# phylovi/libsbn

Measured on AMD Instinct MI355X. Metric: tree log-likelihoods+gradients/sec (batched), higher is better.
Workload: dtype f64; 1 GPU; DS1 27 taxa x 934 site patterns x 1000 trees per step over 1 GPU(s), JC69+weibull+4 (K=4), phylo_gradients: logL + branch + site gradients; trees_total=1000, trees_per_gpu=1000, taxa=27, patterns=934, categories=4, parallelism=single GPU

## Files before the change

libsbn_amd/csrc/kernels_finalize.hip:

```cpp
#include <hip/hip_runtime.h>

#include <algorithm>
#include <cstdlib>
#include <string>

#include "mi_phylo_device_utils.h"
#include "mi_phylo_kernels.h"

namespace miphylo {

namespace {
using namespace dev;

__device__ __forceinline__ void reduce_tiles_body(const ReduceArgs& a, const int b, double* red_lds ,
                                                  double* keep = nullptr) {
  __shared__ double llw[4];
  const int lane = threadIdx.x & 63, wv = threadIdx.x >> 6;
  const int N2 = 2 * a.N;
  const int W = a.g_width ? a.g_width : N2;
  const int t = b < a.T ? b : b - a.T;
  const bool positional = b < a.Eg && a.g_width;
  const int mcount = positional ? a.macro_count[t] : 0;
  double llp = 0;
  for (int i = threadIdx.x; i < a.ll_used.of(b); i += 256) llp += a.ll_part[(size_t)b * a.ll_tiles + i];
// ... 507 lines not shown
    if (a.rooted) finalize_body_t<true, true>(a, t, fin_lds, keep);
    else finalize_body_t<true, false>(a, t, fin_lds, keep);
  } else {
    if (a.rooted) finalize_body_t<false, true>(a, t, fin_lds, keep);
    else finalize_body_t<false, false>(a, t, fin_lds, keep);
  }
}

__global__ __launch_bounds__(64) void finalize_kernel(FinalizeArgs a) {
  extern __shared__ double fin_lds[];
  finalize_body(a, blockIdx.x, fin_lds);
}

__global__ __launch_bounds__(256) void reduce_finalize_kernel(ReduceArgs ra, FinalizeArgs fa) {
  extern __shared__ double rf_lds[];
  if (threadIdx.x == 0 && fa.clear_ready) fa.clear_ready[(size_t)blockIdx.x * kReadyStride] = 0;
  double* keep = rf_lds + ra.keep_offset;
  reduce_tiles_body(ra, blockIdx.x, rf_lds, keep);
  __threadfence_block();
  __syncthreads();
  if (threadIdx.x >= 64) return;
  finalize_body(fa, blockIdx.x, rf_lds, keep);
}

__device__ __forceinline__ double hess_wave_share(const double* src, int W, int g_tiles, int col, int wv) {
  double s0 = 0, s1 = 0;
  int i = wv;
  for (; i + 4 < g_tiles; i += 8) {
    s0 += src[(size_t)i * W + col];
    s1 += src[(size_t)(i + 4) * W + col];
  }
  if (i < g_tiles) s0 += src[(size_t)i * W + col];
  return s0 + s1;
}
__global__ __launch_bounds__(256) void hessian_finalize_kernel(HessFinalizeArgs a) {
  __shared__ double llw[4];
  const int t = blockIdx.x, lane = threadIdx.x & 63, wv = threadIdx.x >> 6;
// ... 92 lines not shown
  hipLaunchKernelGGL(reduce_tiles_kernel, dim3(a.E), dim3(256), sizeof(double) * 4 * W, s, a);
}
static size_t finalize_lds_bytes(const FinalizeArgs& a) {
  return sizeof(double) * (a.rooted ? 22 * (size_t)a.n : 6 * (size_t)a.n);
}
void launch_reduce_finalize(const ReduceArgs& ra_in, const FinalizeArgs& fa_in, hipStream_t s) {
  FinalizeArgs fa = fa_in;
  ReduceArgs ra = ra_in;
  const size_t W = ra.g_width ? ra.g_width : 2 * (size_t)ra.N;
  const size_t fin = finalize_lds_bytes(fa);
  fa.use_lds = fin <= 48 * 1024;
  const size_t work = std::max(sizeof(double) * 4 * W, fa.use_lds ? fin : 0);
  ra.keep_offset = (int)(work / sizeof(double));
  const size_t lds = work + sizeof(double) * (2 * (size_t)ra.N + 1);
  allow_large_lds(reinterpret_cast<const void*>(reduce_finalize_kernel), lds);
  hipLaunchKernelGGL(reduce_finalize_kernel, dim3(fa.T), dim3(256), lds, s, ra, fa);
}
void launch_finalize(const FinalizeArgs& a_in, hipStream_t s) {
  FinalizeArgs a = a_in;
  const size_t lds = sizeof(double) * (a.rooted ? 22 * (size_t)a.n : 6 * (size_t)a.n);
  a.use_lds = lds <= 48 * 1024;
  hipLaunchKernelGGL(finalize_kernel, dim3(a.T), dim3(64), a.use_lds ? lds : 0, s, a);
}

}
```

libsbn_amd/csrc/kernels_setup.hip:

```cpp
#include <hip/hip_runtime.h>

#include <algorithm>
#include <cstdlib>
#include <string>

#include "mi_phylo_device_utils.h"
#include "mi_phylo_kernels.h"
#include "mi_phylo_setup_device.h"
#include "mi_phylo_macro_slots_device.h"

namespace miphylo {

namespace {
using namespace dev;


__global__ __launch_bounds__(64) void tree_setup_kernel(TreeSetupArgs a, ModelSetupArgs ms) {
  if ((int)blockIdx.x >= a.T) {
    model_setup_thread(ms, ((int)blockIdx.x - a.T) * 64 + (int)threadIdx.x);
    return;
  }
  extern __shared__ int32_t ts_lds[];
  const int t = blockIdx.x;
  const int lane = threadIdx.x;
  const int n = a.n, N = 2 * n - 1;
  const int nodes_in = a.rooted ? N : N - 1;
  const int32_t* par_in = a.parent_ids + (size_t)t * (nodes_in - 1);
  int32_t* maxleaf = a.use_lds ? ts_lds : a.scratch + (size_t)t * 13 * N;
  int32_t* cnt = maxleaf + N;
  int32_t* kids = cnt + N;
  int32_t* c0 = kids + 3 * N;
  int32_t* c1 = c0 + N;
  int32_t* label = c1 + N;
  int32_t* slot = label + N;
  int32_t* stack = slot + N;
  int32_t* par = stack + 2 * N;
  __shared__ int ok_flag;
  SchedEntry* sched = a.sched + (size_t)t * (n - 1);
// ... 147 lines not shown
__device__ __forceinline__ uint64_t up_word(int cls, int label, int isz, int mxl) {
  return (1ull << 63) | ((uint64_t)cls << 56) | ((uint64_t)label << 48) | ((uint64_t)isz << 20) | (uint64_t)mxl;
}
__device__ __forceinline__ int up_cls(uint64_t w) { return (int)(w >> 56) & 3; }
__device__ __forceinline__ int up_label(uint64_t w) { return (int)(w >> 48) & 0xff; }
__device__ __forceinline__ int up_isz(uint64_t w) { return (int)(w >> 20) & 0xfffff; }
__device__ __forceinline__ int up_mxl(uint64_t w) { return (int)w & 0xfffff; }
__global__ __launch_bounds__(kSetupMaxThreads) void tree_setup_wg_kernel(TreeSetupArgs a, ModelSetupArgs ms) {
  const int tid = threadIdx.x, nthreads = blockDim.x;
  if ((int)blockIdx.x >= a.T) {
    model_setup_thread(ms, ((int)blockIdx.x - a.T) * nthreads + tid);
    return;
  }
  extern __shared__ int32_t ts_lds[];
  __shared__ int flag_bad, flag_arity, used_max, chunk_tot[64], ok_flag;
  const int t = blockIdx.x;
  const int n = a.n, N = 2 * n - 1;
  const int nodes_in = a.rooted ? N : N - 1, root_in = nodes_in - 1;
  const int32_t* par_in = a.parent_ids + (size_t)t * (nodes_in - 1);
#define TS_LDS(T) volatile __attribute__((address_space(3))) T*
  typedef __attribute__((address_space(3))) int32_t* ts_lds_base;
  const ts_lds_base ts3 = (ts_lds_base)ts_lds;
  TS_LDS(int4) kid = (TS_LDS(int4))ts3;
  TS_LDS(uint64_t) W = (TS_LDS(uint64_t))(ts3 + 4 * N);
  TS_LDS(uint64_t) D = W + N;
  TS_LDS(int2) cc = (TS_LDS(int2))(D + N);
  TS_LDS(int2) up = cc + N;
  TS_LDS(int32_t) par = (TS_LDS(int32_t))(up + N);
  TS_LDS(int32_t) sslot = par + N;
#undef TS_LDS
  int32_t* kid_i = ts_lds;
// ... 248 lines not shown
  if (a.arena_macros) {
    __syncthreads();
    macro_slots_wg_body(ts_lds, a.macros, a.arena_macros, macro_M, n, t, a.slot_need, a.arena_sure, a.status);
  }
}


template <int NB>
__global__ __launch_bounds__(64) void tree_setup_small_kernel(TreeSetupArgs a, ModelSetupArgs ms) {
  if ((int)blockIdx.x >= a.T) {
    model_setup_thread(ms, ((int)blockIdx.x - a.T) * 64 + (int)threadIdx.x);
    return;
  }
  __shared__ int tree_lds[kSmallTreeLdsInts * NB];
  SmallTree<NB> tree;
  small_tree_build<NB>(a, blockIdx.x, threadIdx.x, tree, tree_lds);
  small_tree_store<NB>(a, blockIdx.x, threadIdx.x, tree);
}

constexpr int kTransitionBlock = 256;
__global__ __launch_bounds__(kTransitionBlock) void transition_kernel(TransitionArgs a) {
  __shared__ double stage[kTransitionBlock * 17];
  const long per = (long)a.K * (a.N - 1);
  const long first = (long)blockIdx.x * kTransitionBlock + (long)a.eval_base * per;
  const long idx = first + threadIdx.x;
  const long total = (long)(a.eval_base + a.E) * per;
  {
    const long last = (first + kTransitionBlock - 1 < total ? first + kTransitionBlock - 1 : total - 1);
    if (first / per >= a.ev_skip_begin && last / per < a.ev_skip_end) return;
  }
  if (idx < total) {
    const int k = idx % a.K;
// ... 100 lines not shown
```

libsbn_amd/csrc/mi_phylo_call.cpp:

```cpp
#include "mi_phylo_engine.h"

namespace {

bool use_arena(const mi_engine* e, bool rescale, bool subst, size_t waves = (size_t)-1, int regs = 0) {
  const bool lut = walk3_possible(e) && e->sw.walk3_arena && !subst && gradient_mfma_groups(e->K) == 1;
  return gradient_walk_use_arena(e->sw.gradient_store, e->n, e->K, rescale, subst, waves, lut, regs);
}
bool walk_fits(const mi_engine* e, bool rescale) { return gradient_walk_fits(e->n, e->K, rescale); }

const char* loglik_kernel_of(const mi_engine* e, bool rescaling) {
  LikArgs probe{};
  probe.n = e->n;
  probe.K = e->K;
  probe.tip_masks = e->have_tip_masks ? e->tip_masks.as<uint8_t>() : nullptr;
  return loglik_kernel_name(probe, rescaling, e->max_slots, e->sw);
}
bool matrix_core_gradient(const mi_engine* e, bool rescaling, bool loglik_is_valu) {
  return !e->sw.hbm_gradient && e->have_tip_masks && walk_fits(e, rescaling) &&
         reduce_tiles_fits(e->N) && (gradient_mfma_groups(e->K) == 1 || !loglik_is_valu);
}

size_t plv_bytes_per_eval(const mi_engine* e) {
  return (size_t)(e->n - 1) * e->K * e->tiles * kTile * 4 * sizeof(double);
}
// ... 88 lines not shown
  p.need_slots = !(gradient && p.mfma && p.groups == 1 && (!p.gtr || p.analytic || p.light));
  const bool arena = p.mfma && use_arena(e, rescaling, p.analytic, (size_t)T * (size_t)p.g_tiles, p.tile_regs);
  p.store = !p.mfma ? kStoreHbm : arena ? kStoreArena : kStoreLds;
  p.reserve_arena = p.mfma && (e->tile_regs || use_arena(e, false, true) || use_arena(e, true, true) ||
                               use_arena(e, false, false) || use_arena(e, true, false));
  p.hand_off_words = gradient && e->fused_setup && walk3_possible(e);
  const bool fuse_possible = p.mfma && walk3_possible(e) && !p.analytic && p.groups == 1 && !arena && !p.tile_regs && e->fused_setup &&
                             e->sw.fuse_finalize && p.E == T && p.models_per_tree == 1 && !p.need_slots &&
                             T <= e->sw.fused_max_trees && gradient_walk_lut_fused_applies(n, e->K);
  p.walk3 = p.mfma && walk3_possible(e) && !p.analytic && p.groups == 1 &&
            (p.tile_regs || (arena ? e->sw.walk3_arena : (e->K > 1 || e->sw.walk3_k1_lds || fuse_possible)));
  p.fuse_setup = p.walk3 && fuse_possible;
  p.setup_records = p.walk3 && !p.fuse_setup && !arena && !p.tile_regs && !p.analytic && p.groups == 1 && e->fused_setup &&
                    p.E == T && p.models_per_tree == 1 && !p.need_slots && T <= kMaxEvals &&
                    gradient_walk_lut_fused_applies(n, e->K) && e->sw.setup_records;
  p.fd_pass = gradient && p.gtr && !p.analytic && want_subst;
  p.site_pass = p.site_separate && want_site;
  p.loglik_runs = !gradient || p.fd_pass || (p.mfma && p.groups > 1);
  p.need_tip_tables = p.loglik_runs && p.loglik_is_valu;
  if (gradient)
    p.dominant = p.fuse_setup ? gradient_walk_lut_fused_kernel_name()
                 : p.walk3    ? gradient_walk_lut_kernel_name()
                 : p.mfma     ? gradient_walk_kernel_name()
                              : gradient_kernel_name();
  return p;
}

std::string plan_path(const mi_engine* e, const CallPlan& p) {
  std::string path = p.dominant;
  if (p.kind != kLogLikCall)
    path += p.store == kStoreHbm ? " store=hbm" : (p.store == kStoreArena ? " store=arena" : " store=lds");
  path += p.fuse_setup ? " setup=in-walk" : (p.setup_records ? " setup=with-records" : " setup=own-launch");
  if (p.kind == kHessianCall) path += " hess";
  if (p.kind == kNniCall) path += " nni";
  if (p.tile_regs > kLlR) path += " tile=wide";
  if (p.fd_pass) path += " fd=16";
  if (p.site_pass) path += " site-pass";
  if (p.light) path += " light";
  if (p.analytic) path += " analytic";
  if (p.rescaling) path += " rescaled";
  if (p.rooted) path += " rooted";
  return path + " K=" + std::to_string(e->K);
}

int reserve(mi_engine* e, const CallPlan& p) {
  const int n = e->n, N = e->N, T = p.T;
  const bool gradient = p.kind == kGradientCall;
  if (e->tree_scratch.ensure(sizeof(int32_t) * (size_t)T * 13 * N)) return 1;
  if (e->sched.ensure(sizeof(SchedEntry) * (size_t)T * (n - 1))) return 1;
  if (e->macros.ensure(sizeof(MacroEntry) * (size_t)T * macro_stride(n))) return 1;
  if (e->macro_count.ensure(sizeof(int32_t) * (size_t)T)) return 1;
  if (e->bl_eff.ensure(sizeof(double) * (size_t)T * N)) return 1;
  if (e->models.ensure(sizeof(DevModel) * (size_t)p.M)) return 1;
  if (e->mats.ensure(sizeof(double) * (size_t)p.E * (N - 1) * e->K * 16)) return 1;
  if (e->tip_tables.ensure(sizeof(double) * (size_t)p.E * n * e->K * 20)) return 1;
  if (gradient) {
    if (e->mmats.ensure(p.mmats_bytes_per_eval * (size_t)p.Eg)) return 1;
// ... 194 lines not shown
void macro_slots(const mi_engine* e, int T, hipStream_t s) {
  launch_macro_slots(e->macros.as<MacroEntry>(), e->arena_macros.as<MacroEntry>(),
                     e->macro_count.as<int32_t>(), e->n, T, e->slot_need.as<int32_t>(),
                     e->status.as<int32_t>(), e->sw, s);
}

void note_call(mi_engine* e, const CallPlan& p, int first_launch_evals, int walk_launches) {
  e->dominant = p.dominant;
  e->last_path = plan_path(e, p);
  e->prof_first_launch_evals = first_launch_evals;
  e->last_evals = p.E;
  e->last_grad_evals = p.Eg;
  e->last_walk_launches = walk_launches;
}

int check_call(const mi_engine* e, const DeviceCall& d, const void* output) {
  if (d.T <= 0) return fail("tree_count must be positive");
  if (!d.parent_ids || !d.bl || !output) return fail("null tree / output pointer");
  if (e->param_count > 0 && !d.params) return fail("null parameter matrix");
  return 0;
}

}

int run_device(mi_engine* e, hipStream_t s, const DeviceCall& d) {
  HIP_TRY(hipSetDevice(e->spec.device));
  if (e->s == kAa) return aa_run_device(e, s, d);
  if (check_call(e, d, d.out_ll)) return 1;
  const CallPlan p = plan_call(e, d.gradient ? kGradientCall : kLogLikCall, d);
  if (reserve(e, p)) return 1;
  const int n = e->n, N = e->N, T = d.T;
  const bool prof = e->prof_used < e->prof_capacity;
  const bool marks = prof && e->prof_phases;
  PROF_MARK(e, marks, 0, s);

  if (p.setup_records) launch_setup_records(fused_setup_args(e, d, p), T, s);
  const bool slots_done = !p.fuse_setup && !p.setup_records &&
                          launch_setup(tree_setup_args(e, d, p), model_setup_args(e, d, p), e->sw, s);
  if (p.store == kStoreArena && !slots_done) macro_slots(e, T, s);

  TransitionArgs tr = transition_args(e, d, p);
  if (p.mfma && p.groups == 1) {
    if (p.fd_pass) {
      tr.eval_base = T;
      tr.E = 16 * T;
      launch_transition(tr, s);
    }
  } else {
// ... 38 lines not shown
  PROF_MARK(e, marks, 1, s);
  PROF_MARK(e, marks, 2, s);
  if (!d.gradient) {
    loglik_range(0, T);
    if (prof) HIP_TRY(hipEventRecord(prof_event(e, 1), s));
    PROF_MARK(e, marks, 3, s);
  } else {
    grad_range(0, 0, T);
    if (prof) HIP_TRY(hipEventRecord(prof_event(e, 1), s));
    PROF_MARK(e, marks, 3, s);
    if (p.fd_pass) loglik_range(T, 16 * T);
    if (p.site_pass) grad_range(17 * T, T, T);
  }
  note_call(e, p, T, walk_launches);

  FinalizeArgs fa = finalize_args(e, d);
  fa.ll_tiles = e->ll_stride;
  fa.g_tiles = p.g_tiles;
  fa.ll_part = e->ll_part.as<double>();
  fa.g_part = e->g_part.as<double>();
  const int ll_kernel_count = p.loglik_is_valu ? e->tiles : loglik_mfma_tiles(e->P, e->K);
  const int grad_kernel_count =
      p.mfma ? (p.groups > 1 ? ll_kernel_count : p.g_tiles) : e->tiles;
  LlCounts ll_used{d.gradient ? grad_kernel_count : ll_kernel_count, ll_kernel_count, 0, 0};
  if (d.gradient && p.gtr && !p.analytic && !p.light) {
    ll_used.mid_lo = T;
    ll_used.mid_hi = 17 * T;
  }
  fa.ll_used = ll_used;
  bool fused = false;
  ReduceArgs ra{};
  if (reduce_tiles_fits(N)) {
    ra.N = N;
    ra.E = p.E;
    ra.Eg = p.Eg;
    ra.ll_tiles = e->ll_stride;
    ra.ll_used = ll_used;
    ra.g_tiles = p.g_tiles;
    ra.ll_part = e->ll_part.as<double>();
    ra.g_part = e->g_part.as<double>();
    ra.ll_sum = e->ll_sum.as<double>();
    ra.g_sum = e->g_sum.as<double>();
    ra.g_width = p.mfma ? gradient_mfma_width(n, p.analytic) : 0;
    ra.extra = p.analytic ? kSubstExtra : 0;
    ra.x_sum = e->x_sum.as<double>();
    ra.n = n;
    ra.T = T;
    ra.macros = walk_macros(e, p);
    ra.macro_count = e->macro_count.as<int32_t>();
    fused = e->sw.fuse_finalize && p.E == T;
    if (!fused) launch_reduce_tiles(ra, s);
    fa.ll_tiles = 1;
    fa.ll_used = LlCounts{1, 1, 0, 0};
    fa.g_tiles = 1;
    fa.ll_part = ra.ll_sum;
    fa.g_part = ra.g_sum;
  }
  fa.gtr = p.gtr && !p.analytic && !p.light;
  fa.site_fused = p.site_fused;
  fa.site_separate = p.site_separate;
  fa.out_subst = d.out_subst;
  fa.clear_ready = p.fuse_setup ? e->ready.as<int32_t>() : nullptr;
  if (p.fuse_setup && !fused) return fail("internal error: the one-launch call needs the fused reduction");
  if (fused) launch_reduce_finalize(ra, fa, s);
  else launch_finalize(fa, s);
  if (p.analytic && d.out_subst) {
    SubstGradArgs sg{};
    sg.T = T;
    sg.param_count = e->param_count;
    sg.rates_off = e->rates_off;
    sg.freqs_off = e->freqs_off;
    sg.params = d.params;
    sg.models = e->models.as<DevModel>();
    sg.x_sum = e->x_sum.as<double>();
    sg.out_subst = d.out_subst;
    launch_subst_gradient(sg, s);
  }
// ... 154 lines not shown
```

libsbn_amd/csrc/mi_phylo_engine.cpp:

```cpp
#include <map>

#include "mi_phylo_engine.h"

namespace {
thread_local std::string g_error;
}

namespace miphylo {
int fail(const std::string& msg) {
  g_error = msg;
  return 1;
}
void set_last_error(const std::string& msg) { g_error = msg; }
}

namespace {
int build_tip_tiles(mi_engine* e) {
  e->tile_regs = engine_tile_regs(e);
  if (!e->have_tip_masks || e->K > kMaxCategories) return 0;
  if (e->tip_tiles.ensure(loglik_tip_tiles_bytes(e->n, e->P, e->K))) return 1;
  launch_tip_tiles(e->tip_masks.as<uint8_t>(), e->tip_tiles.as<uint8_t>(), e->n, e->P, e->K, e->stream);
  if (walk3_possible(e) && gradient_mfma_groups(e->K) == 1) {
    const int regs = e->tile_regs;
    if (e->tip_code_tiles.ensure(tip_code_tiles_bytes(e->n, e->P, e->K, regs))) return 1;
// ... 203 lines not shown
    e->clock_off = off;
    add_block(bm, "clock rate", off, 1);
    off += 1;
  }
  add_block(bm, "entire clock", clock_start, off - clock_start);
  add_block(bm, "entire", 0, off);
  e->param_count = off;
  for (const auto& kv : bm) e->blocks.push_back({kv.first, kv.second.first, kv.second.second});

  auto cleanup_fail = [&](int) {
    mi_engine_destroy(e);
    return 1;
  };
  if (hipStreamCreateWithFlags(&e->stream, hipStreamNonBlocking) != hipSuccess)
    return cleanup_fail(fail("hipStreamCreate failed"));
  if (e->status.ensure(sizeof(int32_t) * kStatusWords) ||
      hipMemsetAsync(e->status.ptr, 0, sizeof(int32_t) * kStatusWords, e->stream) != hipSuccess)
    return cleanup_fail(fail("status word allocation failed"));
  if (spec->site_model == MI_SITE_WEIBULL) {
    if (e->weibull_x.ensure(sizeof(double) * 2 * (size_t)e->K)) return cleanup_fail(1);
    launch_weibull_table(e->K, e->weibull_x.as<double>(), e->stream);
  }
  const size_t np = (size_t)e->n * e->P;
  if (device_tips) {
    for (const void* p : {static_cast<const void*>(device_tips), static_cast<const void*>(device_weights)}) {
      hipPointerAttribute_t at{};
      if (hipPointerGetAttributes(&at, p) != hipSuccess || at.type != hipMemoryTypeDevice ||
          at.device != e->spec.device) {
        (void)hipGetLastError();
        return cleanup_fail(fail("device_tip_states / device_pattern_weights must be device memory of "
// ... 113 lines not shown
  if (upload(e->weights, pattern_weights, (size_t)e->P, e->stream)) return cleanup_fail(1);
  if (hipStreamSynchronize(e->stream) != hipSuccess)
    return cleanup_fail(fail("upload of tips failed"));
  *out_engine = e;
  return 0;
}

void mi_engine_destroy(mi_engine* e) {
  if (!e) return;
  for (mi_engine* shard : e->shards) mi_engine_destroy(shard);
  e->shards.clear();
  if (e->stream || e->tip_states.ptr) (void)hipSetDevice(e->spec.device);
  if (e->stream) {
    (void)hipStreamSynchronize(e->stream);
  }
  for (Buffer* b :
       {&e->tip_states, &e->tip_partials, &e->tip_masks, &e->tip_tiles, &e->tip_code_tiles, &e->tip_codes, &e->weights, &e->tree_scratch, &e->sched, &e->macros,
        &e->arena_macros, &e->slot_need,
        &e->macro_count, &e->tip_tables, &e->mmats, &e->mphi, &e->x_sum, &e->bl_eff,
        &e->models, &e->mats, &e->ll_part, &e->plv, &e->g_part, &e->site_lik, &e->site_exp, &e->fin_scratch,
        &e->ll_sum, &e->g_sum, &e->status, &e->ready, &e->weibull_x, &e->aa_model, &e->aa_matP, &e->aa_matPT,
        &e->aa_tipP, &e->aa_tipPQ, &e->aa_exp_cum, &e->aa_exp_loc, &e->aa_root_val,
        &e->aa_root_exp, &e->aa_root_scale, &e->red_ll, &e->red_g, &e->red_site, &e->red_sort,
        &e->in_pack, &e->out_pack, &e->opt_ws})
    b->release();
  if (e->opt_word) (void)hipHostFree(e->opt_word);
  e->pinned.release();
  for (hipEvent_t ev : e->prof_events) (void)hipEventDestroy(ev);
  if (e->stream) (void)hipStreamDestroy(e->stream);
  delete e;
}

int32_t mi_engine_param_count(const mi_engine* e) { return e ? e->param_count : -1; }
int32_t mi_engine_block_count(const mi_engine* e) { return e ? (int32_t)e->blocks.size() : -1; }
int32_t mi_engine_block(const mi_engine* e, int32_t index, const char** name, int32_t* start,
                        int32_t* length) {
  if (!e || index < 0 || index >= (int32_t)e->blocks.size()) return fail("block index out of range");
  if (name) *name = e->blocks[index].name.c_str();
  if (start) *start = e->blocks[index].start;
  if (length) *length = e->blocks[index].length;
  return 0;
}

// ... 449 lines not shown
```

libsbn_amd/csrc/mi_phylo_engine.h:

```cpp
#pragma once
#include <hip/hip_runtime.h>

#include <algorithm>
#include <cstring>
#include <initializer_list>
#include <string>
#include <vector>

#include "../../include/mi_phylo.h"
#include "mi_phylo_kernels.h"

namespace miphylo {
int fail(const std::string& msg);
void set_last_error(const std::string& msg);
}
using miphylo::fail;
using namespace miphylo;

#define HIP_TRY(expr)                                                              \
  do {                                                                             \
    hipError_t err__ = (expr);                                                     \
    if (err__ != hipSuccess)                                                       \
      return fail(std::string("HIP error: ") + hipGetErrorString(err__) + " at " + \
                  __FILE__ + ":" + std::to_string(__LINE__));                      \
// ... 75 lines not shown
    case kNotTrifurcatingRoot:
      return "UnrootedTree::Detrifurcate given a non-trifurcating tree.";
    case kGtrFrequencies: return "GTR frequencies do not sum to 1 +/- 0.001!";
    case kGtrRates: return "GTR rates do not sum to 1 +/- 0.001!";
    case kBadRateCount:
      return "The number of rates should be equal to 1 (i.e. strict clock) or equal to the "
             "number of branches.";
    case kTooManySlots: return "internal error: evaluation schedule needs too many LDS slots";
    case kFusedTimeout:
      return "internal error: the walk waves of the one-launch call waited in vain for their "
             "tree's set-up waves (MI_PHYLO_FUSED_SETUP=0 selects the four-launch sequence)";
    default: return "unknown device status";
  }
}

constexpr int kStatusWords = 4;

struct mi_engine {
  mi_engine_spec spec;
  int n, N, P, K, tiles, max_slots, ll_stride;
  int s = 4;
  int param_count, rates_off, freqs_off, shape_off, clock_off;
  std::vector<Block> blocks;
  hipStream_t stream = nullptr;
  Buffer tip_states, tip_partials, tip_masks, tip_codes, weights;
  Buffer tip_code_tiles;
  Buffer tip_tiles;
  bool have_tip_masks = false;
  bool have_tip_codes = false;
  Buffer arena_macros, slot_need, tree_scratch, sched, macros, macro_count, bl_eff, models, mats, tip_tables, mmats, mphi, x_sum, ll_part, plv, g_part, site_lik, site_exp, fin_scratch,
      ll_sum, g_sum, status;
  Buffer weibull_x;
  Buffer ready;
  bool fused_setup = true;
  bool fused_timed_out = false;
  int fused_fallbacks = 0;
  Buffer aa_model, aa_matP, aa_matPT, aa_tipP, aa_tipPQ, aa_exp_cum, aa_exp_loc,
      aa_root_val, aa_root_exp, aa_root_scale;
  bool aa_reserved_gradient = false;
// ... 38 lines not shown
struct CallPlan {
  CallKind kind;
  int T;
  bool rescaling, rooted;
  int E, Eg, M, models_per_tree;
  bool gtr, site_fused, site_separate;
  bool mfma;
  bool walk3;
  WalkStore store;
  int groups;
  int tile_regs;
  int g_tiles;
  bool analytic;
  bool light;
  bool fuse_setup;
  bool setup_records;
  bool need_slots;
  bool fd_pass, site_pass;
  bool loglik_runs;
  bool loglik_is_valu;
  bool need_tip_tables;
  size_t mmats_bytes_per_eval;
  bool reserve_arena;
  bool hand_off_words;
  const char* dominant;
};
struct DeviceCall {
  bool gradient = false, rooted = false, with_jacobian = false, rescaling = false;
  int T = 0;
  const int32_t* parent_ids = nullptr;
// ... 9 lines not shown
  double* out_ratios = nullptr;
  double* out_clock = nullptr;
  double* out_site = nullptr;
  double* out_subst = nullptr;
  double* out_hess = nullptr;
  double* out_gsq = nullptr;
  double* out_nni = nullptr;
  int32_t* out_best = nullptr;
  int route_T = 0;
};
CallPlan plan_call(const mi_engine* e, CallKind kind, int T, bool rescaling, int route_T = 0,
                   bool rooted = false, bool want_site = true, bool want_subst = true);
inline CallPlan plan_call(const mi_engine* e, CallKind kind, const DeviceCall& d) {
  return plan_call(e, kind, d.T, d.rescaling, d.route_T, d.rooted, d.out_site != nullptr, d.out_subst != nullptr);
}
std::string plan_path(const mi_engine* e, const CallPlan& p);
bool walk3_possible(const mi_engine* e);
int engine_tile_regs(const mi_engine* e);
int reserve(mi_engine* e, const CallPlan& p);
int reserve_hessian(mi_engine* e, const CallPlan& p);
int reserve_hessian_calls(mi_engine* e, int T);
TreeSetupArgs tree_setup_args(const mi_engine* e, const DeviceCall& d, const CallPlan& p);
ModelSetupArgs model_setup_args(const mi_engine* e, const DeviceCall& d, const CallPlan& p);
FinalizeArgs finalize_args(const mi_engine* e, const DeviceCall& d);
int run_device(mi_engine* e, hipStream_t s, const DeviceCall& d);
int run_hessian_device(mi_engine* e, hipStream_t s, const DeviceCall& d);
int reserve_nni(mi_engine* e, const CallPlan& p);
int reserve_nni_calls(mi_engine* e, int T);
int run_nni_device(mi_engine* e, hipStream_t s, const DeviceCall& d);
int32_t nni_best_move(int n, const double* delta);
// ... 36 lines not shown
```

libsbn_amd/csrc/mi_phylo_kernels.h:

```cpp
#pragma once
#include <hip/hip_runtime.h>

#include "mi_phylo_device.h"
#include "mi_phylo_switches.h"

namespace miphylo {

struct EvalMap {
  int T;
  int models_per_tree;
  __host__ __device__ void decode(int e, int& tree, int& model) const {
    if (e < T) {
      tree = e;
      model = e * models_per_tree;
    } else if (e < 17 * T) {
      tree = (e - T) / 16;
      model = tree * kFdModels + 1 + (e - T) % 16;
    } else {
      tree = e - 17 * T;
      model = tree * kFdModels + 16;
    }
  }
};

// ... 2 lines not shown
  const int32_t* parent_ids;
  const double* bl;
  const double* rates;
  int32_t* scratch;
  SchedEntry* sched;
  MacroEntry* macros;
  int32_t* macro_count;
  double* bl_eff;
  int32_t* status;
  int max_slots;
  int use_lds;
  int need_slots;
  MacroEntry* arena_macros;
  int32_t* slot_need;
  int arena_sure;
};

struct ModelSetupArgs {
  int T, models_per_tree;
  int subst, site, K;
  int param_count, rates_off, freqs_off, shape_off;
  const double* params;
  DevModel* models;
  int32_t* status;
  const double* weibull_x;
};

struct TransitionArgs {
  int E, N, K;
  EvalMap map;
  const DevModel* models;
  const double* bl_eff;
  double* mats;
  double* tip_tables;
  int n;
  int ev_skip_begin, ev_skip_end;
  int eval_base;
};

struct TransitionMacroArgs {
// ... 66 lines not shown
  const int32_t* rate_counts;
  const double* node_heights;
  const double* node_bounds;
  const double* height_ratios;
  const SchedEntry* sched;
  double* scratch;
  double* out_ll;
  double* out_branch;
  double* out_ratios;
  double* out_clock;
  double* out_site;
  double* out_subst;
  int32_t* status;
  int use_lds;
  int32_t* clear_ready;
};

bool launch_setup(const TreeSetupArgs& a, const ModelSetupArgs& ms, const Switches& sw, hipStream_t s);
bool launch_tree_setup(const TreeSetupArgs& a, const Switches& sw, hipStream_t s);
void launch_weibull_table(int K, double* table, hipStream_t s);
void launch_transition(const TransitionArgs& a, hipStream_t s);
void launch_loglik(const LikArgs& a, int count, bool rescale, int max_slots, const Switches& sw, hipStream_t s);
int loglik_mfma_tiles(int P, int K);
size_t loglik_tip_tiles_bytes(int n, int P, int K);
void launch_tip_tiles(const uint8_t* masks, uint8_t* tiles, int n, int P, int K, hipStream_t s);
int gradient_mfma_tiles(int P, int K, int regs = 0);
size_t tip_code_tiles_bytes(int n, int P, int K, int regs);
void launch_tip_code_tiles(const uint8_t* codes, uint8_t* out, int n, int P, int K, int regs, hipStream_t s);
int gradient_walk_tile_regs(int n, int P, int K, int forced);
void launch_gradient_hbm(const LikArgs& a, int count, bool rescale, hipStream_t s);
// ... 224 lines not shown
```

libsbn_amd/csrc/mi_phylo_setup_device.h:

```cpp
#pragma once
#include <hip/hip_runtime.h>

#include "mi_phylo_device_utils.h"
#include "mi_phylo_kernels.h"

namespace miphylo {
namespace dev {

#define RDL(arr, i) __builtin_amdgcn_readlane((arr), (i))
#define WRL(arr, i, val) (arr) = (lane == (i)) ? (val) : (arr)
template <int NB>
struct NodeArray {
  int r[NB];
  __device__ __forceinline__ void fill(int v) {
#pragma unroll
    for (int nb = 0; nb < NB; nb++) r[nb] = v;
  }
  __device__ __forceinline__ int rd(int i) const {
    int out = __builtin_amdgcn_readlane(r[0], i & 63);
#pragma unroll
    for (int nb = 1; nb < NB; nb++) {
      const int x = __builtin_amdgcn_readlane(r[nb], i & 63);
      out = (i >> 6) == nb ? x : out;
    }
// ... 582 lines not shown
  for (int i = 0; i < K; i++) {
    mean_rate = __dadd_rn(mean_rate, lane_value(r, i));
    mean_deriv = __dadd_rn(mean_deriv, lane_value(du, i));
  }
  mean_rate = __ddiv_rn(mean_rate, (double)K);
  mean_deriv = __ddiv_rn(mean_deriv, (double)K);
  if (lane < K) {
    weibull_normalise(mean_rate, mean_deriv, r, du);
    m.cat_rate[lane] = r;
    m.cat_drate[lane] = du;
    m.cat_weight[lane] = 1.0 / K;
  }
}
__device__ inline void model_setup_thread(const ModelSetupArgs& a, int idx) {
  if (idx >= a.T * a.models_per_tree) return;
  model_setup_into(a, idx, a.models[idx]);
}

}
}
```

libsbn_amd/csrc/mi_phylo_switches.cpp:

```cpp
#include "mi_phylo_switches.h"

#include <cerrno>
#include <climits>
#include <cstdlib>
#include <cstring>

namespace miphylo {
namespace {

struct Reader {
  std::string error;

  const char* get(const char* name) {
    const char* v = getenv(name);
    return v && *v ? v : nullptr;
  }
  void reject(const char* name, const char* value, const std::string& expected) {
    if (error.empty()) error = std::string(name) + "=" + value + ": expected " + expected;
  }
  int choice(const char* name, const char* values, int dflt) {
    const char* v = get(name);
    if (!v) return dflt;
    const size_t len = strlen(v);
    int index = 0;
// ... 49 lines not shown
  s.arena_nt = r.listed("MI_PHYLO_ARENA_NT", "0|1", -1);
  s.tip_tiles = r.on_off("MI_PHYLO_TIP_TILES", true);
  s.analytic_subst = r.choice("MI_PHYLO_SUBST_GRADIENT", "fd|analytic", 0) == 1;
  s.loglik_path = r.choice("MI_PHYLO_LOGLIK_PATH", "valu|mfma", -1) + 1;
  s.loglik_evals_per_wave = r.listed("MI_PHYLO_LOGLIK_EVALS_PER_WAVE", "1|2|4|8", 0);
  s.tree_setup = r.choice("MI_PHYLO_TREE_SETUP", "small|wg|lds", -1) + 1;
  s.macro_slots = r.choice("MI_PHYLO_MACRO_SLOTS", "own|seq", -1) + 1;
  s.setup_records = r.on_off("MI_PHYLO_SETUP_RECORDS", false);
  s.fused_setup = r.on_off("MI_PHYLO_FUSED_SETUP", true);
  s.fuse_finalize = r.on_off("MI_PHYLO_FUSE_FINALIZE", true);
  s.fused_max_trees = (int)r.integer("MI_PHYLO_FUSED_MAX_TREES", 0, INT_MAX, 512);
  s.fused_fence = r.choice("MI_PHYLO_FUSED_FENCE", "none|l1|agent", 1);
  s.fused_colocate = r.on_off("MI_PHYLO_FUSED_COLOCATE", true);
  s.fused_spin_ticks = (int)(r.number("MI_PHYLO_FUSED_SPIN_MS", 0.01, 2.0e4, "[0.01, 20000]", 0.0) * 1.0e5);
  s.fused_debug_skip = (int)r.integer("MI_PHYLO_DEBUG_FUSED_SKIP", 0, INT_MAX, 0);
  s.plv_bytes = r.integer("MI_PHYLO_PLV_BYTES", 0, LLONG_MAX, -1);
  s.aa_jacobi_seq = r.choice("MI_PHYLO_AA_JACOBI", "wave|seq", 0) == 1;
  s.aa_post_wave = r.choice("MI_PHYLO_AA_POST", "wg|wave", 0) == 1;
  s.aa_pre_wave = r.choice("MI_PHYLO_AA_PRE", "wg|wave", 0) == 1;
  s.aa_post_tiles = r.listed("MI_PHYLO_AA_POST_TILES", "1|2|4", 0);
  s.aa_post_one_tile_below = (long)r.integer("MI_PHYLO_AA_POST_ONE_TILE_BELOW", 0, LONG_MAX, -1);
  s.aa_ring = r.listed("MI_PHYLO_AA_RING", "0|1|2|4", -1);
  s.aa_pre_ring = r.listed("MI_PHYLO_AA_PRE_RING", "0|1|2", -1);
  s.aa_lds_pad = (size_t)r.integer("MI_PHYLO_AA_LDS_PAD", 0, 160 * 1024, 0);
  error = r.error;
  if (!error.empty()) return false;
  out = s;
  return true;
}

// ... 2 lines not shown
```

libsbn_amd/csrc/mi_phylo_switches.h:

```cpp
#pragma once
#include <cstddef>
#include <string>

namespace miphylo {

struct Switches {
  bool hbm_gradient = false;
  bool walk3 = true;
  bool walk3_arena = true;
  bool walk3_k1_lds = true;
  int gradient_store = 0;
  int walk_tile_regs = 0;
  int walk_tiles_per_wave = 0;
  int arena_nt = -1;
  bool tip_tiles = true;
  bool analytic_subst = false;
  int loglik_path = 0;
  int loglik_evals_per_wave = 0;
  int tree_setup = 0;
  int macro_slots = 0;
  bool setup_records = false;
  bool fused_setup = true;
  bool fuse_finalize = true;
  int fused_max_trees = 512;
  int fused_fence = 1;
  bool fused_colocate = true;
  int fused_spin_ticks = 0;
  int fused_debug_skip = 0;
  long long plv_bytes = -1;
  bool aa_jacobi_seq = false;
  bool aa_post_wave = false;
  bool aa_pre_wave = false;
  int aa_post_tiles = 0;
  long aa_post_one_tile_below = -1;
  int aa_ring = -1;
  int aa_pre_ring = -1;
  size_t aa_lds_pad = 0;
};

bool parse_switches(Switches& out, std::string& error);

}
```

Measured before the change: 1.265 million trees/s.

## Pipeline tree batches across two streams to overlap setup, walk and finalize

Splits a large gradient batch into parts of about 128 trees. Each part runs setup, transition, gradient walk and fused reduce-finalize, and consecutive parts alternate between the main stream and a new side stream so one part's serial phases can overlap another's. Kernels take a tree_begin offset so they can work on a sub-range. The change adds launch overhead and event synchronisation, and the overlapping parts compete for compute units.

```diff
diff --git a/libsbn_amd/csrc/kernels_finalize.hip b/libsbn_amd/csrc/kernels_finalize.hip
--- a/libsbn_amd/csrc/kernels_finalize.hip
+++ b/libsbn_amd/csrc/kernels_finalize.hip
@@ -545,13 +545,14 @@
 
 __global__ __launch_bounds__(256) void reduce_finalize_kernel(ReduceArgs ra, FinalizeArgs fa) {
   extern __shared__ double rf_lds[];
-  if (threadIdx.x == 0 && fa.clear_ready) fa.clear_ready[(size_t)blockIdx.x * kReadyStride] = 0;
+  const int t = fa.tree_begin + (int)blockIdx.x;
+  if (threadIdx.x == 0 && fa.clear_ready) fa.clear_ready[(size_t)t * kReadyStride] = 0;
   double* keep = rf_lds + ra.keep_offset;
-  reduce_tiles_body(ra, blockIdx.x, rf_lds, keep);
+  reduce_tiles_body(ra, t, rf_lds, keep);
   __threadfence_block();
   __syncthreads();
   if (threadIdx.x >= 64) return;
-  finalize_body(fa, blockIdx.x, rf_lds, keep);
+  finalize_body(fa, t, rf_lds, keep);
 }
 
 __device__ __forceinline__ double hess_wave_share(const double* src, int W, int g_tiles, int col, int wv) {
@@ -674,7 +675,7 @@
   ra.keep_offset = (int)(work / sizeof(double));
   const size_t lds = work + sizeof(double) * (2 * (size_t)ra.N + 1);
   allow_large_lds(reinterpret_cast<const void*>(reduce_finalize_kernel), lds);
-  hipLaunchKernelGGL(reduce_finalize_kernel, dim3(fa.T), dim3(256), lds, s, ra, fa);
+  hipLaunchKernelGGL(reduce_finalize_kernel, dim3(fa.tree_count ? fa.tree_count : fa.T), dim3(256), lds, s, ra, fa);
 }
 void launch_finalize(const FinalizeArgs& a_in, hipStream_t s) {
   FinalizeArgs a = a_in;
diff --git a/libsbn_amd/csrc/kernels_setup.hip b/libsbn_amd/csrc/kernels_setup.hip
--- a/libsbn_amd/csrc/kernels_setup.hip
+++ b/libsbn_amd/csrc/kernels_setup.hip
@@ -21,7 +21,7 @@
     return;
   }
   extern __shared__ int32_t ts_lds[];
-  const int t = blockIdx.x;
+  const int t = a.tree_begin + (int)blockIdx.x;
   const int lane = threadIdx.x;
   const int n = a.n, N = 2 * n - 1;
   const int nodes_in = a.rooted ? N : N - 1;
@@ -199,7 +199,7 @@
   }
   extern __shared__ int32_t ts_lds[];
   __shared__ int flag_bad, flag_arity, used_max, chunk_tot[64], ok_flag;
-  const int t = blockIdx.x;
+  const int t = a.tree_begin + (int)blockIdx.x;
   const int n = a.n, N = 2 * n - 1;
   const int nodes_in = a.rooted ? N : N - 1, root_in = nodes_in - 1;
   const int32_t* par_in = a.parent_ids + (size_t)t * (nodes_in - 1);
@@ -478,8 +478,9 @@
   }
   __shared__ int tree_lds[kSmallTreeLdsInts * NB];
   SmallTree<NB> tree;
-  small_tree_build<NB>(a, blockIdx.x, threadIdx.x, tree, tree_lds);
-  small_tree_store<NB>(a, blockIdx.x, threadIdx.x, tree);
+  const int t = a.tree_begin + (int)blockIdx.x;
+  small_tree_build<NB>(a, t, threadIdx.x, tree, tree_lds);
+  small_tree_store<NB>(a, t, threadIdx.x, tree);
 }
 
 constexpr int kTransitionBlock = 256;
diff --git a/libsbn_amd/csrc/mi_phylo_call.cpp b/libsbn_amd/csrc/mi_phylo_call.cpp
--- a/libsbn_amd/csrc/mi_phylo_call.cpp
+++ b/libsbn_amd/csrc/mi_phylo_call.cpp
@@ -126,6 +126,23 @@
   p.setup_records = p.walk3 && !p.fuse_setup && !arena && !p.tile_regs && !p.analytic && p.groups == 1 && e->fused_setup &&
                     p.E == T && p.models_per_tree == 1 && !p.need_slots && T <= kMaxEvals &&
                     gradient_walk_lut_fused_applies(n, e->K) && e->sw.setup_records;
+  p.parts = 1;
+  p.part_size = 0;
+  const bool phases = e->prof_phases && e->prof_used < e->prof_capacity;
+  if (gradient && e->sw.pipeline && p.walk3 && p.store == kStoreLds && !p.tile_regs && !p.fuse_setup &&
+      !p.setup_records && !rooted && p.E == T && p.models_per_tree == 1 && T > e->sw.fused_max_trees && T <= kMaxEvals &&
+      e->sw.fuse_finalize && reduce_tiles_fits(e->N) && !phases) {
+    const long long min_waves =
+        e->sw.pipeline_min_waves >= 0
+            ? e->sw.pipeline_min_waves
+            : 4ll * device_compute_units() * gradient_walk_waves_per_cu(kStoreLds, n, e->K);
+    if ((long long)T * p.g_tiles >= min_waves) {
+      p.part_size = e->sw.pipeline_part;
+      int begin = 0;
+      for (p.parts = 0; begin < T; p.parts++) begin += plan_part(p, p.parts, begin);
+      if (p.parts < 2) p.parts = 1;
+    }
+  }
   p.fd_pass = gradient && p.gtr && !p.analytic && want_subst;
   p.site_pass = p.site_separate && want_site;
   p.loglik_runs = !gradient || p.fd_pass || (p.mfma && p.groups > 1);
@@ -136,6 +153,11 @@
                  : p.mfma     ? gradient_walk_kernel_name()
                               : gradient_kernel_name();
   return p;
+}
+
+int plan_part(const CallPlan& p, int i, int& begin) {
+  const int size = i == 1 ? std::max(8, (p.part_size / 2 + 7) / 8 * 8) : p.part_size;
+  return std::min(size, p.T - begin);
 }
 
 std::string plan_path(const mi_engine* e, const CallPlan& p) {
@@ -152,7 +174,9 @@
   if (p.analytic) path += " analytic";
   if (p.rescaling) path += " rescaled";
   if (p.rooted) path += " rooted";
-  return path + " K=" + std::to_string(e->K);
+  path += " K=" + std::to_string(e->K);
+  if (p.parts > 1) path += " parts=" + std::to_string(p.parts);
+  return path;
 }
 
 int reserve(mi_engine* e, const CallPlan& p) {
@@ -377,10 +401,103 @@
   e->last_walk_launches = walk_launches;
 }
 
+bool reduce_finalize_args(const mi_engine* e, const DeviceCall& d, const CallPlan& p, ReduceArgs& ra, FinalizeArgs& fa) {
+  const int n = e->n, N = e->N, T = d.T;
+  fa = finalize_args(e, d);
+  fa.ll_tiles = e->ll_stride;
+  fa.g_tiles = p.g_tiles;
+  fa.ll_part = e->ll_part.as<double>();
+  fa.g_part = e->g_part.as<double>();
+  const int ll_kernel_count = p.loglik_is_valu ? e->tiles : loglik_mfma_tiles(e->P, e->K);
+  const int grad_kernel_count =
+      p.mfma ? (p.groups > 1 ? ll_kernel_count : p.g_tiles) : e->tiles;
+  LlCounts ll_used{d.gradient ? grad_kernel_count : ll_kernel_count, ll_kernel_count, 0, 0};
+  if (d.gradient && p.gtr && !p.analytic && !p.light) {
+    ll_used.mid_lo = T;
+    ll_used.mid_hi = 17 * T;
+  }
+  fa.ll_used = ll_used;
+  bool fused = false;
+  ra = ReduceArgs{};
+  if (reduce_tiles_fits(N)) {
+    ra.N = N;
+    ra.E = p.E;
+    ra.Eg = p.Eg;
+    ra.ll_tiles = e->ll_stride;
+    ra.ll_used = ll_used;
+    ra.g_tiles = p.g_tiles;
+    ra.ll_part = e->ll_part.as<double>();
+    ra.g_part = e->g_part.as<double>();
+    ra.ll_sum = e->ll_sum.as<double>();
+    ra.g_sum = e->g_sum.as<double>();
+    ra.g_width = p.mfma ? gradient_mfma_width(n, p.analytic) : 0;
+    ra.extra = p.analytic ? kSubstExtra : 0;
+    ra.x_sum = e->x_sum.as<double>();
+    ra.n = n;
+    ra.T = T;
+    ra.macros = walk_macros(e, p);
+    ra.macro_count = e->macro_count.as<int32_t>();
+    fused = e->sw.fuse_finalize && p.E == T;
+    fa.ll_tiles = 1;
+    fa.ll_used = LlCounts{1, 1, 0, 0};
+    fa.g_tiles = 1;
+    fa.ll_part = ra.ll_sum;
+    fa.g_part = ra.g_sum;
+  }
+  fa.gtr = p.gtr && !p.analytic && !p.light;
+  fa.site_fused = p.site_fused;
+  fa.site_separate = p.site_separate;
+  fa.out_subst = d.out_subst;
+  fa.clear_ready = p.fuse_setup ? e->ready.as<int32_t>() : nullptr;
+  return fused;
+}
+
 int check_call(const mi_engine* e, const DeviceCall& d, const void* output) {
   if (d.T <= 0) return fail("tree_count must be positive");
   if (!d.parent_ids || !d.bl || !output) return fail("null tree / output pointer");
   if (e->param_count > 0 && !d.params) return fail("null parameter matrix");
+  return 0;
+}
+
+int run_parts(mi_engine* e, hipStream_t s, const DeviceCall& d, const CallPlan& p, bool prof) {
+  const PipeEvents& ev = e->pipe_events[e->pipe_next];
+  e->pipe_next = (e->pipe_next + 1) % kPipeEventSets;
+  const hipStream_t side = e->side_stream;
+  HIP_TRY(hipEventRecord(ev.fork, s));
+  HIP_TRY(hipStreamWaitEvent(side, ev.fork, 0));
+  if (prof) HIP_TRY(hipEventRecord(prof_event(e, 0), s));
+  TreeSetupArgs ts = tree_setup_args(e, d, p);
+  ModelSetupArgs ms = model_setup_args(e, d, p);
+  const LikArgs la = lik_args(e, d, p);
+  ReduceArgs ra{};
+  FinalizeArgs fa{};
+  if (!reduce_finalize_args(e, d, p, ra, fa)) return fail("internal error: the pipelined call needs the fused reduction");
+  int begin = 0;
+  for (int i = 0; i < p.parts; i++) {
+    const int count = plan_part(p, i, begin);
+    const hipStream_t chain = (p.parts - 1 - i) & 1 ? side : s;
+    ts.tree_begin = ms.tree_begin = begin;
+    ts.T = ms.T = count;
+    launch_setup(ts, ms, e->sw, chain);
+    launch_transition_lut(transition_macro_args(e, d, p, begin, begin, count), chain);
+    LikArgs g = la;
+    g.eval_offset = g.grad_offset = begin;
+    launch_gradient_walk_lut(g, count, d.rescaling, e->sw, chain);
+    if (prof && i == p.parts - 2) HIP_TRY(hipEventRecord(ev.walks, chain));
+    if (prof && i == p.parts - 1) {
+      HIP_TRY(hipStreamWaitEvent(chain, ev.walks, 0));
+      HIP_TRY(hipEventRecord(prof_event(e, 1), chain));
+    }
+    fa.tree_begin = begin;
+    fa.tree_count = count;
+    launch_reduce_finalize(ra, fa, chain);
+    begin += count;
+  }
+  HIP_TRY(hipEventRecord(ev.join, side));
+  HIP_TRY(hipStreamWaitEvent(s, ev.join, 0));
+  note_call(e, p, plan_part(p, 0, begin = 0), p.parts);
+  if (prof) e->prof_used++;
+  HIP_TRY(hipGetLastError());
   return 0;
 }
 
@@ -392,9 +509,10 @@
   if (check_call(e, d, d.out_ll)) return 1;
   const CallPlan p = plan_call(e, d.gradient ? kGradientCall : kLogLikCall, d);
   if (reserve(e, p)) return 1;
-  const int n = e->n, N = e->N, T = d.T;
+  const int N = e->N, T = d.T;
   const bool prof = e->prof_used < e->prof_capacity;
   const bool marks = prof && e->prof_phases;
+  if (p.parts > 1) return run_parts(e, s, d, p, prof);
   PROF_MARK(e, marks, 0, s);
 
   if (p.setup_records) launch_setup_records(fused_setup_args(e, d, p), T, s);
@@ -463,53 +581,10 @@
   }
   note_call(e, p, T, walk_launches);
 
-  FinalizeArgs fa = finalize_args(e, d);
-  fa.ll_tiles = e->ll_stride;
-  fa.g_tiles = p.g_tiles;
-  fa.ll_part = e->ll_part.as<double>();
-  fa.g_part = e->g_part.as<double>();
-  const int ll_kernel_count = p.loglik_is_valu ? e->tiles : loglik_mfma_tiles(e->P, e->K);
-  const int grad_kernel_count =
-      p.mfma ? (p.groups > 1 ? ll_kernel_count : p.g_tiles) : e->tiles;
-  LlCounts ll_used{d.gradient ? grad_kernel_count : ll_kernel_count, ll_kernel_count, 0, 0};
-  if (d.gradient && p.gtr && !p.analytic && !p.light) {
-    ll_used.mid_lo = T;
-    ll_used.mid_hi = 17 * T;
-  }
-  fa.ll_used = ll_used;
-  bool fused = false;
   ReduceArgs ra{};
-  if (reduce_tiles_fits(N)) {
-    ra.N = N;
-    ra.E = p.E;
-    ra.Eg = p.Eg;
-    ra.ll_tiles = e->ll_stride;
-    ra.ll_used = ll_used;
-    ra.g_tiles = p.g_tiles;
-    ra.ll_part = e->ll_part.as<double>();
-    ra.g_part = e->g_part.as<double>();
-    ra.ll_sum = e->ll_sum.as<double>();
-    ra.g_sum = e->g_sum.as<double>();
-    ra.g_width = p.mfma ? gradient_mfma_width(n, p.analytic) : 0;
-    ra.extra = p.analytic ? kSubstExtra : 0;
-    ra.x_sum = e->x_sum.as<double>();
-    ra.n = n;
-    ra.T = T;
-    ra.macros = walk_macros(e, p);
-    ra.macro_count = e->macro_count.as<int32_t>();
-    fused = e->sw.fuse_finalize && p.E == T;
-    if (!fused) launch_reduce_tiles(ra, s);
-    fa.ll_tiles = 1;
-    fa.ll_used = LlCounts{1, 1, 0, 0};
-    fa.g_tiles = 1;
-    fa.ll_part = ra.ll_sum;
-    fa.g_part = ra.g_sum;
-  }
-  fa.gtr = p.gtr && !p.analytic && !p.light;
-  fa.site_fused = p.site_fused;
-  fa.site_separate = p.site_separate;
-  fa.out_subst = d.out_subst;
-  fa.clear_ready = p.fuse_setup ? e->ready.as<int32_t>() : nullptr;
+  FinalizeArgs fa{};
+  const bool fused = reduce_finalize_args(e, d, p, ra, fa);
+  if (!fused && reduce_tiles_fits(N)) launch_reduce_tiles(ra, s);
   if (p.fuse_setup && !fused) return fail("internal error: the one-launch call needs the fused reduction");
   if (fused) launch_reduce_finalize(ra, fa, s);
   else launch_finalize(fa, s);
diff --git a/libsbn_amd/csrc/mi_phylo_engine.cpp b/libsbn_amd/csrc/mi_phylo_engine.cpp
--- a/libsbn_amd/csrc/mi_phylo_engine.cpp
+++ b/libsbn_amd/csrc/mi_phylo_engine.cpp
@@ -241,6 +241,12 @@
   };
   if (hipStreamCreateWithFlags(&e->stream, hipStreamNonBlocking) != hipSuccess)
     return cleanup_fail(fail("hipStreamCreate failed"));
+  if (hipStreamCreateWithFlags(&e->side_stream, hipStreamNonBlocking) != hipSuccess)
+    return cleanup_fail(fail("hipStreamCreate failed"));
+  for (PipeEvents& pe : e->pipe_events)
+    for (hipEvent_t* ev : {&pe.fork, &pe.walks, &pe.join})
+      if (hipEventCreateWithFlags(ev, hipEventDisableTiming) != hipSuccess)
+        return cleanup_fail(fail("hipEventCreate failed"));
   if (e->status.ensure(sizeof(int32_t) * kStatusWords) ||
       hipMemsetAsync(e->status.ptr, 0, sizeof(int32_t) * kStatusWords, e->stream) != hipSuccess)
     return cleanup_fail(fail("status word allocation failed"));
@@ -384,6 +390,7 @@
   if (e->stream) {
     (void)hipStreamSynchronize(e->stream);
   }
+  if (e->side_stream) (void)hipStreamSynchronize(e->side_stream);
   for (Buffer* b :
        {&e->tip_states, &e->tip_partials, &e->tip_masks, &e->tip_tiles, &e->tip_code_tiles, &e->tip_codes, &e->weights, &e->tree_scratch, &e->sched, &e->macros,
         &e->arena_macros, &e->slot_need,
@@ -397,6 +404,10 @@
   if (e->opt_word) (void)hipHostFree(e->opt_word);
   e->pinned.release();
   for (hipEvent_t ev : e->prof_events) (void)hipEventDestroy(ev);
+  for (PipeEvents& pe : e->pipe_events)
+    for (hipEvent_t ev : {pe.fork, pe.walks, pe.join})
+      if (ev) (void)hipEventDestroy(ev);
+  if (e->side_stream) (void)hipStreamDestroy(e->side_stream);
   if (e->stream) (void)hipStreamDestroy(e->stream);
   delete e;
 }
diff --git a/libsbn_amd/csrc/mi_phylo_engine.h b/libsbn_amd/csrc/mi_phylo_engine.h
--- a/libsbn_amd/csrc/mi_phylo_engine.h
+++ b/libsbn_amd/csrc/mi_phylo_engine.h
@@ -113,6 +113,13 @@
   }
 }
 
+constexpr int kPipeEventSets = 8;
+struct PipeEvents {
+  hipEvent_t fork = nullptr;
+  hipEvent_t walks = nullptr;
+  hipEvent_t join = nullptr;
+};
+
 constexpr int kStatusWords = 4;
 
 struct mi_engine {
@@ -122,6 +129,9 @@
   int param_count, rates_off, freqs_off, shape_off, clock_off;
   std::vector<Block> blocks;
   hipStream_t stream = nullptr;
+  hipStream_t side_stream = nullptr;
+  PipeEvents pipe_events[kPipeEventSets];
+  int pipe_next = 0;
   Buffer tip_states, tip_partials, tip_masks, tip_codes, weights;
   Buffer tip_code_tiles;
   Buffer tip_tiles;
@@ -190,6 +200,8 @@
   bool analytic;
   bool light;
   bool fuse_setup;
+  int parts;
+  int part_size;
   bool setup_records;
   bool need_slots;
   bool fd_pass, site_pass;
@@ -229,6 +241,7 @@
 inline CallPlan plan_call(const mi_engine* e, CallKind kind, const DeviceCall& d) {
   return plan_call(e, kind, d.T, d.rescaling, d.route_T, d.rooted, d.out_site != nullptr, d.out_subst != nullptr);
 }
+int plan_part(const CallPlan& p, int i, int& begin);
 std::string plan_path(const mi_engine* e, const CallPlan& p);
 bool walk3_possible(const mi_engine* e);
 int engine_tile_regs(const mi_engine* e);
diff --git a/libsbn_amd/csrc/mi_phylo_kernels.h b/libsbn_amd/csrc/mi_phylo_kernels.h
--- a/libsbn_amd/csrc/mi_phylo_kernels.h
+++ b/libsbn_amd/csrc/mi_phylo_kernels.h
@@ -40,6 +40,7 @@
   MacroEntry* arena_macros;
   int32_t* slot_need;
   int arena_sure;
+  int tree_begin;
 };
 
 struct ModelSetupArgs {
@@ -50,6 +51,7 @@
   DevModel* models;
   int32_t* status;
   const double* weibull_x;
+  int tree_begin;
 };
 
 struct TransitionArgs {
@@ -146,6 +148,7 @@
   int32_t* status;
   int use_lds;
   int32_t* clear_ready;
+  int tree_begin, tree_count;
 };
 
 bool launch_setup(const TreeSetupArgs& a, const ModelSetupArgs& ms, const Switches& sw, hipStream_t s);
diff --git a/libsbn_amd/csrc/mi_phylo_setup_device.h b/libsbn_amd/csrc/mi_phylo_setup_device.h
--- a/libsbn_amd/csrc/mi_phylo_setup_device.h
+++ b/libsbn_amd/csrc/mi_phylo_setup_device.h
@@ -620,6 +620,7 @@
 }
 __device__ inline void model_setup_thread(const ModelSetupArgs& a, int idx) {
   if (idx >= a.T * a.models_per_tree) return;
+  idx += a.tree_begin * a.models_per_tree;
   model_setup_into(a, idx, a.models[idx]);
 }
 
diff --git a/libsbn_amd/csrc/mi_phylo_switches.cpp b/libsbn_amd/csrc/mi_phylo_switches.cpp
--- a/libsbn_amd/csrc/mi_phylo_switches.cpp
+++ b/libsbn_amd/csrc/mi_phylo_switches.cpp
@@ -87,6 +87,10 @@
   s.fused_colocate = r.on_off("MI_PHYLO_FUSED_COLOCATE", true);
   s.fused_spin_ticks = (int)(r.number("MI_PHYLO_FUSED_SPIN_MS", 0.01, 2.0e4, "[0.01, 20000]", 0.0) * 1.0e5);
   s.fused_debug_skip = (int)r.integer("MI_PHYLO_DEBUG_FUSED_SKIP", 0, INT_MAX, 0);
+  s.pipeline = r.on_off("MI_PHYLO_PIPELINE", true);
+  s.pipeline_part = (int)r.integer("MI_PHYLO_PIPELINE_PART", 8, 32768, 128);
+  if (s.pipeline_part % 8) r.reject("MI_PHYLO_PIPELINE_PART", r.get("MI_PHYLO_PIPELINE_PART"), "a multiple of 8");
+  s.pipeline_min_waves = r.integer("MI_PHYLO_PIPELINE_MIN_WAVES", 0, LLONG_MAX, -1);
   s.plv_bytes = r.integer("MI_PHYLO_PLV_BYTES", 0, LLONG_MAX, -1);
   s.aa_jacobi_seq = r.choice("MI_PHYLO_AA_JACOBI", "wave|seq", 0) == 1;
   s.aa_post_wave = r.choice("MI_PHYLO_AA_POST", "wg|wave", 0) == 1;
diff --git a/libsbn_amd/csrc/mi_phylo_switches.h b/libsbn_amd/csrc/mi_phylo_switches.h
--- a/libsbn_amd/csrc/mi_phylo_switches.h
+++ b/libsbn_amd/csrc/mi_phylo_switches.h
@@ -27,6 +27,9 @@
   bool fused_colocate = true;
   int fused_spin_ticks = 0;
   int fused_debug_skip = 0;
+  bool pipeline = true;
+  int pipeline_part = 128;
+  long long pipeline_min_waves = -1;
   long long plv_bytes = -1;
   bool aa_jacobi_seq = false;
   bool aa_post_wave = false;
```

Result: slower. 1.056 million trees/s (-16.5%).
